# Eric-qi/NeuroQuant

Measured on AMD Instinct MI355X. Metric: calibration iters/sec (HNeRV Bunny 1280x640, 21k iters) + final PSNR vs ref, higher is better.
Workload: dtype f32 operands split into bf16 hi+lo, 3 BF16 MFMAs per product, fp32 accumulate (bf16x3); fp32 MFMA on small layers; 1 GPU; HNeRV Bunny_1280x640_3M, channel_wise, bits 6 5 4 5 5 6 6, phase-2 (AdaRound) iteration; per_gpu_batch=2, global_batch=2, frames=132, parallelism=dp1

## Files before the change

include/nq_hip.h:

```cpp
#ifndef NQ_HIP_H
#define NQ_HIP_H

#include <stdint.h>

#ifdef __cplusplus
extern "C" {
#endif

typedef void* nq_stream_t;

#define NQ_API __attribute__((visibility("default")))

#define NQ_OK 0
#define NQ_ERR_INVALID (-1)
#define NQ_ERR_UNSUPPORTED (-2)
#define NQ_ERR_LAUNCH (-3)

NQ_API int nq_abi_version(void);
NQ_API const char* nq_error_string(int code);


NQ_API int nq_scale_init_max(const float* x, int64_t rows, int64_t row_len, int n_levels, float* delta, float* zp,
                      nq_stream_t stream);

// ... 162 lines not shown
  float* db;
  int Cout, N, co_pad, n_pad, nsplit;
  int swap_kk;
  int sg;
} nq_wgr_seg;
NQ_API int nq_conv_wgrad3_slabs(const float* x, const float* dy, float* dw, float* db, float* ws, int B, int Cin, int H, int W, int Cout,
                         int k, nq_wgr_seg* seg, nq_stream_t stream);
NQ_API int nq_conv_wgrad3_slabs_fmt(const float* x, const float* dy, float* dw, float* db, float* ws, int B, int Cin, int H, int W,
                             int Cout, int k, nq_wgr_seg* seg, int fmt, nq_stream_t stream);
NQ_API int nq_conv_wgrad3_swapped_slabs(const float* x, const float* dy, float* dw, float* ws, int B, int Cin, int H, int W, int Cout,
                                 int k, nq_wgr_seg* seg, nq_stream_t stream);
NQ_API int nq_conv_wgrad_slabs(const float* x, const float* dy, float* dw, float* db, float* ws, int B, int Cin, int H, int W, int Cout,
                        int k, int x_gelu, nq_wgr_seg* seg, nq_stream_t stream);
NQ_API int nq_wgrad_reduce_multi(const nq_wgr_seg* segs, int nseg, nq_stream_t stream);

NQ_API int nq_ps_gelu_backward(const float* da, const float* z, float* dconv, int B, int C, int H, int W, int r,
                        nq_stream_t stream);

NQ_API int nq_tanh_out_backward(const float* dimg, const float* img, float* dconv, int64_t n, nq_stream_t stream);

NQ_API int nq_l2_loss(const float* pred, const float* tgt, float* loss, float* dpred, float* ws, int64_t n, int64_t mean_count,
               float gscale, nq_stream_t stream);

NQ_API int nq_channel_sum(const float* x, float* out, float* ws, int B, int C, int64_t HW, nq_stream_t stream);

NQ_API int nq_l2_loss_tanh_head(const float* pred, const float* tgt, const uint8_t* cache_u8, const int64_t* idx, float* loss,
                         float* dconv, float* db, float* ws, int B, int C, int64_t HW, int64_t mean_count, float gscale,
                         nq_stream_t stream);

NQ_API int64_t nq_head_forward_loss_ws_floats(int B, int H, int W);
// ... 22 lines not shown
```

neuroquant_amd/_lib.py:

```python
import ctypes
import os
from ctypes import c_char_p, c_float, c_int, c_int64, c_void_p, POINTER, Structure

_HERE = os.path.dirname(os.path.abspath(__file__))
LIB_PATH = os.environ.get("NQ_LIB") or os.path.join(_HERE, "libnqhip.so")

NQ_OK = 0
ABI_VERSION = 5
EPI_PLAIN, EPI_PS_GELU, EPI_TANH, EPI_PS, EPI_DGRAD_GELU = 0, 1, 2, 3, 4


class NQLibraryError(RuntimeError):
    pass


class AdaSeg(Structure):
    _fields_ = [("x", c_void_p), ("gy", c_void_p), ("alpha", c_void_p), ("delta", c_void_p), ("zp", c_void_p),
                ("out", c_void_p), ("rows", c_int64), ("row_len", c_int64), ("per_row", c_int), ("n_levels", c_int),
                ("soft", c_int), ("reg_weight", c_float)]


class WL3Seg(Structure):
    _fields_ = [("w", c_void_p), ("wt3", c_void_p), ("Cin", c_int), ("Cout", c_int), ("k", c_int), ("transposed", c_int)]

# ... 86 lines not shown
    sig("nq_weight_layout3", I, P, P, I, I, I, I, P)
    sig("nq_weight_layout3_multi", I, POINTER(WL3Seg), I, P)
    sig("nq_weight_layouts_multi", I, POINTER(WLSeg), I, P)
    sig("nq_weight_layouts_all", I, POINTER(WL3Seg), I, POINTER(WLSeg), I, P)
    sig("nq_conv_forward3_ws_floats", L, I, I, I, I, I, I)
    sig("nq_conv_forward3", I, P, P, P, P, P, P, P, I, I, I, I, I, I, I, I, P)
    sig("nq_conv_wgrad3_supported", I, I, I, I, I, I, I)
    sig("nq_conv_wgrad3_ws_floats", L, I, I, I, I, I, I)
    sig("nq_conv_wgrad3_plan", I, I, I, I, I, I, I, POINTER(c_int), POINTER(c_int), POINTER(c_int), POINTER(c_int))
    sig("nq_conv_wgrad3", I, P, P, P, P, P, I, I, I, I, I, I, P)
    sig("nq_conv_wgrad3_swapped", I, P, P, P, P, I, I, I, I, I, I, P)
    sig("nq_conv_wgrad3_slabs", I, P, P, P, P, P, I, I, I, I, I, I, POINTER(WgrSeg), P)
    sig("nq_conv_wgrad3_swapped_slabs", I, P, P, P, P, I, I, I, I, I, I, POINTER(WgrSeg), P)
    sig("nq_conv_wgrad_slabs", I, P, P, P, P, P, I, I, I, I, I, I, I, POINTER(WgrSeg), P)
    sig("nq_wgrad_reduce_multi", I, POINTER(WgrSeg), I, P)
    sig("nq_conv_wgrad_ws_floats", L, I, I, I, I, I, I)
    sig("nq_conv_wgrad", I, P, P, P, P, P, I, I, I, I, I, I, I, P)
    sig("nq_ps_gelu_backward", I, P, P, P, I, I, I, I, I, P)
    sig("nq_tanh_out_backward", I, P, P, P, L, P)
    sig("nq_l2_loss", I, P, P, P, P, P, L, L, F, P)
    sig("nq_channel_sum", I, P, P, P, I, I, L, P)
    sig("nq_l2_loss_tanh_head", I, P, P, P, P, P, P, P, P, I, I, L, L, F, P)
    sig("nq_frame_sse", I, P, P, P, L, L, P)
    sig("nq_ms_ssim_ws_floats", L, L, I, I, I)
    sig("nq_ms_ssim", I, P, P, P, P, L, I, I, I, P)
    sig("nq_gather_frames_u8", I, P, P, P, L, L, P)
    sig("nq_adaround_fwht_multi", I, POINTER(FqFwhtSeg), I, P)
    sig("nq_fwht_adaround_adam_multi", I, POINTER(FqFwhtSeg), I, F, F, F, F, F, F, P, P)
    sig("nq_head_forward_loss_ws_floats", L, I, I, I)
    sig("nq_head_forward_loss", I, P, P, I, P, P, P, P, P, P, P, P, P, I, I, I, I, L, F, P)
# ... 3 lines not shown
    return lib


EXPORTS = (
    "nq_abi_version", "nq_error_string", "nq_scale_init_max", "nq_uaq_forward", "nq_uaq_backward",
    "nq_adaround_init", "nq_adaround_forward", "nq_adaround_backward", "nq_reduce_ws_floats", "nq_round_loss", "nq_round_loss_backward",
    "nq_adam_step", "nq_adaround_adam_multi", "nq_adaround_forward_multi", "nq_uaq_forward_multi", "nq_uaq_backward_multi", "nq_adaround_backward_multi", "nq_adam_step_multi", "nq_step_prologue", "nq_step_prologue_gather", "nq_adaround_backward_multi_dyn", "nq_adam_step_multi_dyn", "nq_fwht", "nq_fwht_multi", "nq_weight_layouts", "nq_conv_operand_dims", "nq_conv_forward_ws_floats", "nq_conv_forward",
    "nq_conv3_supported", "nq_conv3_weight_bytes", "nq_weight_layout3", "nq_weight_layout3_multi", "nq_weight_layouts_multi", "nq_conv_forward3_ws_floats", "nq_conv_forward3",
    "nq_conv_wgrad3_supported", "nq_conv_wgrad3_ws_floats", "nq_conv_wgrad3_plan", "nq_conv_wgrad3", "nq_conv_wgrad3_swapped",
    "nq_conv_wgrad3_slabs", "nq_conv_wgrad3_swapped_slabs", "nq_conv_wgrad_slabs", "nq_wgrad_reduce_multi",
    "nq_conv_wgrad_ws_floats", "nq_conv_wgrad", "nq_ps_gelu_backward", "nq_tanh_out_backward", "nq_l2_loss",
    "nq_channel_sum", "nq_l2_loss_tanh_head", "nq_frame_sse", "nq_ms_ssim_ws_floats", "nq_ms_ssim", "nq_gather_frames_u8",
    "nq_act_dd", "nq_pixel_shuffle", "nq_bias_add", "nq_conv3_split_io", "nq_conv_split_out", "nq_split_words",
    "nq_conv_wgrad3_split_io", "nq_conv_wgrad3_fmt", "nq_conv_wgrad3_slabs_fmt", "nq_head_forward_loss_ws_floats", "nq_head_forward_loss",
    "nq_adaround_fwht_multi", "nq_fwht_adaround_adam_multi", "nq_weight_layouts_all",
)

_lib = None


def lib():
    global _lib
    if _lib is None:
        _lib = _load()
    return _lib


def check(rc, what=""):
    if rc != NQ_OK:
        msg = lib().nq_error_string(rc).decode()
# ... 2 lines not shown
```

neuroquant_amd/csrc/conv.hip:

```cpp
#include <algorithm>

#include "nq_common.h"

extern "C" {
int nq_tiny_pw_supported(int B, int Cin, int H, int W, int Cout, int k);
int nq_tiny_pw_forward(const float* x, const float* wt, const float* bias, float* y, float* z, const float* zprev, int B,
                       int Cin, int H, int W, int Cout, int ld, int r, int epi, hipStream_t st);
int nq_tiny_pw_wgrad(const float* x, const float* dy, float* dw, float* db, int B, int Cin, int H, int W, int Cout,
                     hipStream_t st);
}

extern "C" {
int nq_conv_igemm_k1(const float*, const float*, const float*, float*, float*, int, int, int, int, int, int, int, int, int,
                     int, float*, int, const float*, hipStream_t);
int nq_conv_igemm_k3(const float*, const float*, const float*, float*, float*, int, int, int, int, int, int, int, int, int,
                     int, float*, int, const float*, hipStream_t);
int nq_conv_igemm_k5(const float*, const float*, const float*, float*, float*, int, int, int, int, int, int, int, int, int,
                     int, float*, int, const float*, hipStream_t);
int nq_conv_splitk_finish(const float*, const float*, float*, float*, const float*, int, int, int, int, int, int, int,
                          hipStream_t);
int nq_head_supported(int, int);
int nq_head_forward(const float*, const float*, int, const float*, float*, int, int, int, int, int, int, int, hipStream_t);
int nq_head_dgrad(const float*, const float*, int, const float*, float*, int, int, int, int, int, int, int, int, hipStream_t);
int nq_head_dgrad_streams(int, int, int, int, int, int, int, int);
// ... 256 lines not shown
  const int mi = pick_mi_fwd(Cout);
  const int ns = pick_nsplit(B, Cin, H, W, Cout, k);
  if (ns > 1 && !ws) return NQ_ERR_INVALID;
  if ((int64_t)B * ns > 65535) return NQ_ERR_UNSUPPORTED;
  hipStream_t st = nq_s(stream);
  int rc;
  switch (k) {
    case 1: rc = nq_conv_igemm_k1(x, wt, bias, y, z, B, Cin, H, W, Cout, ld, r, epilogue, mi, ns, ws, in_gelu, zprev, st); break;
    case 3: rc = nq_conv_igemm_k3(x, wt, bias, y, z, B, Cin, H, W, Cout, ld, r, epilogue, mi, ns, ws, in_gelu, zprev, st); break;
    default: rc = nq_conv_igemm_k5(x, wt, bias, y, z, B, Cin, H, W, Cout, ld, r, epilogue, mi, ns, ws, in_gelu, zprev, st); break;
  }
  if (rc != NQ_OK || ns == 1) return rc;
  return nq_conv_splitk_finish(ws, bias, y, z, zprev, B, H, W, Cout, r, epilogue, ns, st);
}

int64_t nq_conv_wgrad_ws_floats(int B, int Cin, int H, int W, int Cout, int k) {
  if (!ks_ok(k) || B <= 0 || Cin <= 0 || H <= 0 || W <= 0 || Cout <= 0) return 0;
  WgradPlan p = plan_wgrad(B, Cin, H, W, Cout, k);
  return (int64_t)p.nsplit * p.co_pad * ((int64_t)p.n_pad + 1);
}

static int conv_wgrad_impl(const float* x, const float* dy, float* dw, float* db, float* ws, int B, int Cin, int H, int W,
                           int Cout, int k, int x_gelu, nq_wgr_seg* seg, nq_stream_t stream);

int nq_conv_wgrad(const float* x, const float* dy, float* dw, float* db, float* ws, int B, int Cin, int H, int W, int Cout,
                  int k, int x_gelu, nq_stream_t stream) {
  return conv_wgrad_impl(x, dy, dw, db, ws, B, Cin, H, W, Cout, k, x_gelu, nullptr, stream);
}

int nq_conv_wgrad_slabs(const float* x, const float* dy, float* dw, float* db, float* ws, int B, int Cin, int H, int W, int Cout,
// ... 36 lines not shown
```

neuroquant_amd/csrc/conv3.hip:

```cpp
#include <cstdlib>
#include "nq_common.h"
#include "conv3_layout.h"

extern "C" {
int nq_conv_igemm3_k3(const float*, const void*, const float*, float*, float*, const float*, int, int, int, int, int, int, int,
                      int, int, int, float*, hipStream_t);
int nq_conv_igemm3_k5(const float*, const void*, const float*, float*, float*, const float*, int, int, int, int, int, int, int,
                      int, int, int, float*, hipStream_t);
int nq_conv_splitk_finish(const float*, const float*, float*, float*, const float*, int, int, int, int, int, int, int, hipStream_t);
int nq_conv3_nst_k3();
int nq_conv3_nst_k5();
int nq_conv3_nst8_k3();
int nq_conv3_nst8_k5();
int nq_conv3_nstk_k3(int);
int nq_conv3_nstk_k5(int);
int nq_conv_flat3_plan(int, int, int, int, int, int, int*, int*, int*, int*);
int nq_conv_flat3(const float*, const void*, const float*, float*, float*, const float*, float*, int, int, int, int, int, int, int, int,
                  int, int, int, int, hipStream_t);
int nq_conv_wgrad_flat3_ok(int, int, int, int, int, int);
int nq_conv_wgrad_flat3(const float*, const float*, float*, float*, int, int, int, int, int, int, hipStream_t);
int nq_conv_wgrad3_k3(const float*, const float*, float*, float*, int, int, int, int, int, int, int, int, int, int, int, int, hipStream_t);
int nq_conv_wgrad3_k5(const float*, const float*, float*, float*, int, int, int, int, int, int, int, int, int, int, int, int, hipStream_t);
}

namespace {

constexpr int CC = 16;

inline int pick_mi3(int Cout) {
  if (Cout <= 16) return 1;
  if (Cout <= 32) return 2;
  int best = 3, best_pad = 1 << 30;
  for (int mi = 5; mi >= 3; --mi) {
    int mt = 16 * mi, pad = (Cout + mt - 1) / mt * mt;
    if (pad < best_pad) {
// ... 289 lines not shown
      } else {
        dw[i] = t;
      }
    } else if (db && i < total + Cout) {
      db[(int)(i - total)] = t;
    }
  }
}

constexpr int WGR_MAXSEG = 16;
struct WGRMulti {
  nq_wgr_seg s[WGR_MAXSEG];
  int blk0[WGR_MAXSEG + 1];
  int nseg;
};
__global__ __launch_bounds__(256) void wgrad_reduce_multi_kernel(WGRMulti t) {
  __shared__ float4 part[256];
  int k = 0;
  while (k + 1 < t.nseg && (int)blockIdx.x >= t.blk0[k + 1]) ++k;
  const nq_wgr_seg& q = t.s[k];
  const int SG = q.sg, OG = 256 / SG;
  const int o = threadIdx.x % OG, g = threadIdx.x / OG;
  const int N = q.N, Cout = q.Cout, nsplit = q.nsplit;
  const int NQ = (N + 3) >> 2;
  const int64_t i = (int64_t)((int)blockIdx.x - t.blk0[k]) * OG + o;
  const int64_t total = (int64_t)Cout * NQ;
  float4 s = make_float4(0.f, 0.f, 0.f, 0.f);
  int co = 0, n = 0;
  if (i < total) {
    co = (int)(i / NQ);
    n = 4 * (int)(i - (int64_t)co * NQ);
    const float* p = q.slab + (int64_t)co * q.n_pad + n;
    const int64_t stride = (int64_t)q.co_pad * q.n_pad;
#pragma unroll 8
    for (int j = g; j < nsplit; j += SG) {
      const float4 v = *reinterpret_cast<const float4*>(p + j * stride);
      s.x += v.x; s.y += v.y; s.z += v.z; s.w += v.w;
    }
  } else if (q.db && i < total + Cout) {
    const int cb = (int)(i - total);
// ... 17 lines not shown
      for (int e = 0; e < 4; ++e) {
        if (n + e >= N) break;
        const int ci = (n + e) / q.swap_kk, tap = (n + e) - ci * q.swap_kk;
        q.dw[((int64_t)ci * Cout + co) * q.swap_kk + (q.swap_kk - 1 - tap)] = sv[e];
      }
    } else if ((N & 3) == 0) {
      *reinterpret_cast<float4*>(q.dw + (int64_t)co * N + n) = s;
    } else {
#pragma unroll
      for (int e = 0; e < 4; ++e)
        if (n + e < N) q.dw[(int64_t)co * N + n + e] = sv[e];
    }
  } else if (q.db && i < total + Cout) {
    q.db[(int)(i - total)] = s.x;
  }
}

}

extern "C" {

int nq_conv3_supported(int B, int Cin, int H, int W, int Cout, int k) {
  if (!(k == 3 || k == 5) || B <= 0 || Cin <= 0 || Cout <= 4 || Cin <= 4) return 0;
  if ((int64_t)B * Cin * H * W * 4 >= 0xFFFFFF00ll) return 0;
  if (use_flat3(B, Cin, H, W, Cout, k, nullptr) && (int64_t)Cin * k * k * Cout >= 65536) return 1;
  const Fwd3Plan p = plan_fwd3(B, Cin, H, W, Cout);
  return p.wgs * p.nsplit >= 128;
}

int64_t nq_conv_forward3_ws_floats(int B, int Cin, int H, int W, int Cout, int k) {
// ... 181 lines not shown
  return conv_wgrad3_impl(dy, x, dw, nullptr, ws, B, Cout, H, W, Cin, k, k * k, nullptr, stream);
}

int nq_conv_wgrad3_slabs(const float* x, const float* dy, float* dw, float* db, float* ws, int B, int Cin, int H, int W, int Cout,
                         int k, nq_wgr_seg* seg, nq_stream_t stream) {
  if (!seg) return NQ_ERR_INVALID;
  return conv_wgrad3_impl(x, dy, dw, db, ws, B, Cin, H, W, Cout, k, 0, seg, stream);
}

int nq_conv_wgrad3_swapped_slabs(const float* x, const float* dy, float* dw, float* ws, int B, int Cin, int H, int W, int Cout,
                                 int k, nq_wgr_seg* seg, nq_stream_t stream) {
  if (!seg) return NQ_ERR_INVALID;
  return conv_wgrad3_impl(dy, x, dw, nullptr, ws, B, Cout, H, W, Cin, k, k * k, seg, stream);
}

int nq_wgrad_reduce_multi(const nq_wgr_seg* segs, int nseg, nq_stream_t stream) {
  if (!segs || nseg < 0) return NQ_ERR_INVALID;
  WGRMulti t;
  t.nseg = 0;
  int blocks = 0;
  auto flush = [&]() {
    if (t.nseg == 0) return;
    t.blk0[t.nseg] = blocks;
    hipLaunchKernelGGL(wgrad_reduce_multi_kernel, dim3((unsigned)blocks), dim3(256), 0, nq_s(stream), t);
    t.nseg = 0;
    blocks = 0;
  };
  for (int i = 0; i < nseg; ++i) {
    const nq_wgr_seg& h = segs[i];
    if (h.nsplit == 0) continue;
    if (!h.slab || !h.dw || h.Cout <= 0 || h.N <= 0 || h.nsplit < 0 || !(h.sg == 1 || h.sg == 4 || h.sg == 16) ||
        (h.db && !h.slab_db))
      return NQ_ERR_INVALID;
    if (t.nseg == WGR_MAXSEG) flush();
    t.s[t.nseg] = h;
    t.blk0[t.nseg] = blocks;
    const int og = 256 / h.sg;
    blocks += (int)(((int64_t)h.Cout * ((h.N + 3) / 4) + h.Cout + og - 1) / og);
    ++t.nseg;
  }
  flush();
  return nq_launch_status();
}

static int conv_wgrad3_impl(const float* x, const float* dy, float* dw, float* db, float* ws, int B, int Cin, int H, int W,
                            int Cout, int k, int swap_kk, nq_wgr_seg* seg, nq_stream_t stream, int fmt) {
  if (!x || !dy || !dw || !ws || B <= 0 || Cin <= 0 || H <= 0 || W <= 0 || Cout <= 0) return NQ_ERR_INVALID;
  if (!(k == 3 || k == 5)) return NQ_ERR_UNSUPPORTED;
  if ((int64_t)Cout * H * W >= (1ll << 31) || (int64_t)Cin * H * W >= (1ll << 31)) return NQ_ERR_UNSUPPORTED;
  if (swap_kk == 0 && nq_conv_wgrad_flat3_ok(B, Cin, H, W, Cout, k)) {
    if (fmt) return NQ_ERR_UNSUPPORTED;
    if (seg) *seg = nq_wgr_seg{nullptr, nullptr, dw, db, Cout, Cin * k * k, 0, 0, 0, 0, 1};
    return nq_conv_wgrad_flat3(x, dy, dw, db, B, Cin, H, W, Cout, k, nq_s(stream));
  }
  if (swap_kk != 0 && nq_conv_wgrad_flat3_ok(B, Cin, H, W, Cout, k)) return NQ_ERR_UNSUPPORTED;
// ... 26 lines not shown
```

neuroquant_amd/csrc/conv_tiny.hip:

```cpp
#include "nq_common.h"

namespace {

template <int KSL>
__global__ __launch_bounds__(256) void tiny_pw_fwd_kernel(const float* __restrict__ x, const float* __restrict__ wt,
                                                          const float* __restrict__ bias, float* __restrict__ y,
                                                          float* __restrict__ z, const float* __restrict__ zprev, int B,
                                                          int Cin, int H, int W, int Cout, int ld, int r, int epi) {
  constexpr int OPB = 256 / KSL;
  __shared__ float part[KSL][OPB];
  const int HW = H * W;
  const int o = threadIdx.x % OPB, ks = threadIdx.x / OPB;
  const int64_t t = (int64_t)blockIdx.x * OPB + o;
  const bool live = t < (int64_t)B * HW * Cout;
  const int co = live ? (int)(t % Cout) : 0, bp = live ? (int)(t / Cout) : 0;
  const int b = bp / HW, p = bp - b * HW;
  const float* __restrict__ xp = x + (int64_t)b * Cin * HW + p;
  float acc = 0.f;
#pragma unroll 8
  for (int ci = ks; ci < Cin; ci += KSL) acc = fmaf(wt[(int64_t)ci * ld + co], xp[(int64_t)ci * HW], acc);
  if (KSL > 1) {
    part[ks][o] = acc;
    __syncthreads();
    if (ks != 0) return;
    acc = part[0][o];
#pragma unroll
    for (int j = 1; j < KSL; ++j) acc += part[j][o];
  }
  if (!live) return;
  float v = acc + (bias ? bias[co] : 0.f);
  const int py = p / W, px = p - py * W;
  if (epi == NQ_EPI_PS_GELU || epi == NQ_EPI_PS) {
    const int rr = r * r, C = Cout / rr;
    const int c = co / rr, rem = co - c * rr, si = rem / r, sj = rem - si * r;
    const int64_t o = (((int64_t)b * C + c) * (H * r) + (int64_t)py * r + si) * ((int64_t)W * r) + (int64_t)px * r + sj;
    if (epi == NQ_EPI_PS_GELU) {
      float gv, dv;
      nq_gelu_pair(v, gv, dv);
      y[o] = gv;
      z[o] = dv;
    } else {
      z[o] = v;
    }
  } else if (epi == NQ_EPI_DGRAD_GELU) {
    const int64_t i = ((int64_t)b * Cout + co) * HW + p;
    v *= zprev[i];
    if (r == 1) {
      y[i] = v;
    } else {
      const int rr = r * r, yq = py / r, xq = px / r;
      const int ch = co * rr + (py - yq * r) * r + (px - xq * r);
      y[(((int64_t)b * Cout * rr + ch) * (H / r) + yq) * (int64_t)(W / r) + xq] = v;
    }
  } else {
    const int64_t i = ((int64_t)b * Cout + co) * HW + p;
    y[i] = (epi == NQ_EPI_TANH) ? tanhf(v) * 0.5f + 0.5f : v;
  }
}

__global__ __launch_bounds__(256) void tiny_pw_wgrad_kernel(const float* __restrict__ x, const float* __restrict__ dy,
                                                            float* __restrict__ dw, float* __restrict__ db, int B, int Cin,
                                                            int HW, int Cout) {
  const int64_t t = (int64_t)blockIdx.x * 256 + threadIdx.x;
  const int64_t nw = (int64_t)Cout * Cin;
  if (t < nw) {
    const int co = (int)(t / Cin), ci = (int)(t - (int64_t)co * Cin);
    float acc = 0.f;
    for (int b = 0; b < B; ++b) {
      const float* __restrict__ dp = dy + ((int64_t)b * Cout + co) * HW;
      const float* __restrict__ xp = x + ((int64_t)b * Cin + ci) * HW;
      if ((HW & 7) == 0) {
        for (int p = 0; p < HW; p += 8) {
          const float4 d0 = *reinterpret_cast<const float4*>(dp + p), d1 = *reinterpret_cast<const float4*>(dp + p + 4);
          const float4 x0 = *reinterpret_cast<const float4*>(xp + p), x1 = *reinterpret_cast<const float4*>(xp + p + 4);
          acc = fmaf(d0.x, x0.x, acc); acc = fmaf(d0.y, x0.y, acc); acc = fmaf(d0.z, x0.z, acc); acc = fmaf(d0.w, x0.w, acc);
          acc = fmaf(d1.x, x1.x, acc); acc = fmaf(d1.y, x1.y, acc); acc = fmaf(d1.z, x1.z, acc); acc = fmaf(d1.w, x1.w, acc);
        }
      } else {
        for (int p = 0; p < HW; ++p) acc = fmaf(dp[p], xp[p], acc);
      }
    }
    dw[t] = acc;
  } else if (db && t < nw + Cout) {
    const int co = (int)(t - nw);
    float acc = 0.f;
    for (int b = 0; b < B; ++b) {
      const float* __restrict__ dp = dy + ((int64_t)b * Cout + co) * HW;
      for (int p = 0; p < HW; ++p) acc += dp[p];
    }
    db[co] = acc;
  }
}

}

extern "C" {

int nq_tiny_pw_supported(int B, int Cin, int H, int W, int Cout, int k) {
  return k == 1 && (int64_t)B * H * W <= 256 && (int64_t)B * H * W * Cout < (1ll << 31);
}

int nq_tiny_pw_forward(const float* x, const float* wt, const float* bias, float* y, float* z, const float* zprev, int B,
                       int Cin, int H, int W, int Cout, int ld, int r, int epi, hipStream_t st) {
  const int64_t total = (int64_t)B * H * W * Cout;
  if (Cin > 1024)
    hipLaunchKernelGGL(tiny_pw_fwd_kernel<64>, dim3((unsigned)((total + 3) / 4)), dim3(256), 0, st, x, wt, bias, y, z, zprev,
                       B, Cin, H, W, Cout, ld, r, epi);
  else if (Cin > 256)
    hipLaunchKernelGGL(tiny_pw_fwd_kernel<16>, dim3((unsigned)((total + 15) / 16)), dim3(256), 0, st, x, wt, bias, y, z, zprev,
                       B, Cin, H, W, Cout, ld, r, epi);
  else if (Cin > 48)
    hipLaunchKernelGGL(tiny_pw_fwd_kernel<4>, dim3((unsigned)((total + 63) / 64)), dim3(256), 0, st, x, wt, bias, y, z, zprev,
                       B, Cin, H, W, Cout, ld, r, epi);
  else
    hipLaunchKernelGGL(tiny_pw_fwd_kernel<1>, dim3((unsigned)((total + 255) / 256)), dim3(256), 0, st, x, wt, bias, y, z, zprev,
                       B, Cin, H, W, Cout, ld, r, epi);
  return nq_launch_status();
}

int nq_tiny_pw_wgrad(const float* x, const float* dy, float* dw, float* db, int B, int Cin, int H, int W, int Cout,
                     hipStream_t st) {
  const int64_t total = (int64_t)Cout * Cin + (db ? Cout : 0);
  hipLaunchKernelGGL(tiny_pw_wgrad_kernel, dim3((unsigned)((total + 255) / 256)), dim3(256), 0, st, x, dy, dw, db, B, Cin,
                     H * W, Cout);
  return nq_launch_status();
}

}
```

neuroquant_amd/ops.py:

```python
import contextlib
import ctypes
import functools
import math
import os
import threading

import torch
from torch.autograd import Function

from . import _lib as L

_QCACHE = {}


def _q(name, *args):
    key = (name, args, os.environ.get("NQ_WGRAD3_PC"), os.environ.get("NQ_WGRAD3_SS"))
    v = _QCACHE.get(key)
    if v is None:
        v = _QCACHE[key] = getattr(L.lib(), name)(*args)
    return v

EPI_PLAIN, EPI_PS_GELU, EPI_TANH, EPI_PS, EPI_DGRAD_GELU = (L.EPI_PLAIN, L.EPI_PS_GELU, L.EPI_TANH, L.EPI_PS,
                                                                L.EPI_DGRAD_GELU)
EPI_X_SPLIT, EPI_Y_SPLIT = 0x100, 0x200


def _stream():
# ... 589 lines not shown
    ws = torch.empty(nws, device=x.device, dtype=torch.float32) if nws else None
    _timed(("conv_igemm3", k, cin, cout, H, W, B, epilogue),
           lambda: L.check(L.lib().nq_conv_forward3(_p(x), _p(wt3), _p(bias), _p(y), _p(z), _p(zprev), _p(ws), B, cin, H, W,
                                                    cout, k, r, epilogue | fmt, _stream()), "conv_forward3"))
    return y, z


def conv_wgrad3_supported(B, cin, H, W, cout, k):
    return bool(_q("nq_conv_wgrad3_supported", B, cin, H, W, cout, k))


class PendingReductions:

    def __init__(self):
        self.segs, self.keep = [], []

    def add(self, seg, *tensors):
        self.segs.append(seg)
        self.keep.append(tensors)

    def flush(self):
        if self.segs:
            arr = (L.WgrSeg * len(self.segs))(*self.segs)
            L.check(L.lib().nq_wgrad_reduce_multi(arr, len(self.segs), _stream()), "wgrad_reduce_multi")
        self.segs, self.keep = [], []


def conv_wgrad3_raw(x, dy, cout, k, want_db, out=None, defer=None, fmt=0):
    B, cin, H, W = x.shape
    ws = torch.empty(_q("nq_conv_wgrad3_ws_floats", B, cin, H, W, cout, k), device=x.device, dtype=torch.float32)
    dw = torch.empty((cout, cin, k, k), device=x.device, dtype=torch.float32) if out is None else out[0]
    db = (torch.empty(cout, device=x.device, dtype=torch.float32) if out is None else out[1]) if want_db else None
    if defer is not None:
        seg = L.WgrSeg()
        _timed(("conv_wgrad3", k, cin, cout, H, W, B, 0),
               lambda: L.check(L.lib().nq_conv_wgrad3_slabs_fmt(_p(x), _p(dy), _p(dw), _p(db), _p(ws), B, cin, H, W, cout, k,
                                                                ctypes.byref(seg), fmt, _stream()), "conv_wgrad3_slabs"))
# ... 28 lines not shown
        _timed(("conv_wgrad3", k, cout, cin, H, W, B, 0),
               lambda: L.check(L.lib().nq_conv_wgrad3_swapped_slabs(_p(x), _p(dy), _p(dw), _p(ws), B, cin, H, W, cout, k,
                                                                    ctypes.byref(seg), _stream()), "conv_wgrad3_swapped_slabs"))
        defer.add(seg, ws, dw)
    else:
        _timed(("conv_wgrad3", k, cout, cin, H, W, B, 0),
               lambda: L.check(L.lib().nq_conv_wgrad3_swapped(_p(x), _p(dy), _p(dw), _p(ws), B, cin, H, W, cout, k, _stream()),
                               "conv_wgrad3_swapped"))
    db = None
    if want_db:
        db = channel_sum(dy)
        if out is not None:
            out[1].copy_(db)
            db = out[1]
    return dw, db


def conv_wgrad_raw(x, dy, cout, k, want_db, x_gelu=False, out=None, defer=None):
    B, cin, H, W = x.shape
    ws = torch.empty(_q("nq_conv_wgrad_ws_floats", B, cin, H, W, cout, k), device=x.device, dtype=torch.float32)
    dw = torch.empty((cout, cin, k, k), device=x.device, dtype=torch.float32) if out is None else out[0]
    db = (torch.empty(cout, device=x.device, dtype=torch.float32) if out is None else out[1]) if want_db else None
    if defer is not None:
        seg = L.WgrSeg()
        _timed(("conv_wgrad", k, cin, cout, H, W, B, 0),
               lambda: L.check(L.lib().nq_conv_wgrad_slabs(_p(x), _p(dy), _p(dw), _p(db), _p(ws), B, cin, H, W, cout, k,
                                                           1 if x_gelu else 0, ctypes.byref(seg), _stream()), "conv_wgrad_slabs"))
        defer.add(seg, ws, dw, db)
        return dw, db
    _timed(("conv_wgrad", k, cin, cout, H, W, B, 0),
# ... 577 lines not shown
    def dgrad(l, dconv):
        k, r, act, cout, cin, in_gelu, wbk, dims_b, has_b, W3, x_split, g_split = metas[l]
        kp, rp, actp = spec.layers[l - 1]
        epi_b, r_b, zp = (EPI_DGRAD_GELU, rp, zs[l]) if actp else (EPI_PLAIN, 1, None)
        if not actp and rp != 1:
            raise NotImplementedError("PixelShuffle without activation between decoder layers")
        out_split = EPI_Y_SPLIT if metas[l - 1][11] else 0
        if W3 is not None:
            d, _ = conv3_forward_raw(dconv, W3, None, cin, k, epi_b, r_b, zprev=zp, fmt=(EPI_X_SPLIT if g_split else 0) | out_split)
        else:
            d, _ = conv_forward_raw(dconv, wbk, dims_b, None, cin, k, epi_b, r_b, zprev=zp, fmt=out_split)
        if not actp and l == 1 and spec.fc_hw != (1, 1):
            d = _channels_from_space(d, *spec.fc_hw).contiguous()
        return d

    def emb_grad(dconv):
        k, r, act, cout, cin, in_gelu, wbk, dims_b, has_b, W3 = metas[0][:10]
        return conv_forward_raw(dconv, wbk, dims_b, None, cin, k, EPI_PLAIN, 1)[0]

    if arena is not None and arena_two_phase and n > 1:
        dcs = [None] * n
        dcs[n - 1] = dconv
        for l in range(n - 1, 0, -1):
            dcs[l - 1] = dgrad(l, dcs[l])
        if ctx.needs_input_grad[0]:
            d_emb = emb_grad(dcs[0])
        flops = [metas[l][3] * metas[l][4] * metas[l][0] ** 2 * xs[l].shape[2] * xs[l].shape[3] for l in range(n)]
        split, late = n - 1, flops[n - 1]
        while split > 1 and late < 0.8 * sum(flops):
            split -= 1
# ... 2 lines not shown
            grads[2 * l], grads[2 * l + 1] = wgrad(l, dcs[l])
            dcs[l] = None
        off = sum(sizes[:2 * split])
        if pending is not None:
            pending.flush()
        yield arena[:off], False
        for l in range(split, n):
            grads[2 * l], grads[2 * l + 1] = wgrad(l, dcs[l])
            dcs[l] = None
        if pending is not None:
            pending.flush()
        yield arena[off:], True
        ctx.nq_arena_reduced = True
        return (d_emb, None) + tuple(grads)

    for l in range(n - 1, -1, -1):
        if side is not None:
            keep.append(dconv)
            side.wait_stream(main)
            with torch.cuda.stream(side):
                dw, db = wgrad(l, dconv)
            for t in (dw, db):
                if t is not None:
                    t.record_stream(main)
        else:
            dw, db = wgrad(l, dconv)
        grads[2 * l], grads[2 * l + 1] = dw, db
        if l == 0:
            if ctx.needs_input_grad[0]:
                d_emb = emb_grad(dconv)
            break
# ... 162 lines not shown
```

Baseline: 501.8 it/s (B=2 frames per iteration-equivalent, summed over GPUs).

## Fuse tiny pointwise dgrad with wgrad and fold first-layer wgrad into reduce

Adds a combined kernel that runs the tiny pointwise conv data-gradient and weight-gradient as separate block ranges of one launch. It also appends the first layer's tiny wgrad blocks onto the deferred slab-reduction kernel. Device bodies are moved into a shared header so several kernels can reuse them. The goal is fewer kernel launches and less serialization in the backward pass for small layers. The fused path is on by default behind an env flag and falls back when unsupported.

New measurement: 504.6 it/s (B=2 frames per iteration-equivalent, summed over GPUs), median of 3. About the same (+0.6%).

```diff
diff --git a/include/nq_hip.h b/include/nq_hip.h
--- a/include/nq_hip.h
+++ b/include/nq_hip.h
@@ -200,6 +200,13 @@
                         int k, int x_gelu, nq_wgr_seg* seg, nq_stream_t stream);
 NQ_API int nq_wgrad_reduce_multi(const nq_wgr_seg* segs, int nseg, nq_stream_t stream);
 
+NQ_API int nq_tiny_pw_supported(int B, int Cin, int H, int W, int Cout, int k);
+NQ_API int nq_conv_dgrad_wgrad_tiny(const float* x, const float* dy, float* dw, float* db, const float* wt_bwd, int krows, int ld,
+                             float* dx, const float* zprev, int B, int Cin, int H, int W, int Cout, int k, int r, int epilogue,
+                             nq_stream_t stream);
+NQ_API int nq_wgrad_reduce_multi_tiny(const nq_wgr_seg* segs, int nseg, const float* x, const float* dy, float* dw, float* db, int B,
+                               int Cin, int H, int W, int Cout, nq_stream_t stream);
+
 NQ_API int nq_ps_gelu_backward(const float* da, const float* z, float* dconv, int B, int C, int H, int W, int r,
                         nq_stream_t stream);
 
diff --git a/neuroquant_amd/_lib.py b/neuroquant_amd/_lib.py
--- a/neuroquant_amd/_lib.py
+++ b/neuroquant_amd/_lib.py
@@ -124,6 +124,9 @@
     sig("nq_conv_wgrad3_swapped_slabs", I, P, P, P, P, I, I, I, I, I, I, POINTER(WgrSeg), P)
     sig("nq_conv_wgrad_slabs", I, P, P, P, P, P, I, I, I, I, I, I, I, POINTER(WgrSeg), P)
     sig("nq_wgrad_reduce_multi", I, POINTER(WgrSeg), I, P)
+    sig("nq_tiny_pw_supported", I, I, I, I, I, I, I)
+    sig("nq_conv_dgrad_wgrad_tiny", I, P, P, P, P, P, I, I, P, P, I, I, I, I, I, I, I, I, P)
+    sig("nq_wgrad_reduce_multi_tiny", I, POINTER(WgrSeg), I, P, P, P, P, I, I, I, I, I, P)
     sig("nq_conv_wgrad_ws_floats", L, I, I, I, I, I, I)
     sig("nq_conv_wgrad", I, P, P, P, P, P, I, I, I, I, I, I, I, P)
     sig("nq_ps_gelu_backward", I, P, P, P, I, I, I, I, I, P)
@@ -157,6 +160,7 @@
     "nq_act_dd", "nq_pixel_shuffle", "nq_bias_add", "nq_conv3_split_io", "nq_conv_split_out", "nq_split_words",
     "nq_conv_wgrad3_split_io", "nq_conv_wgrad3_fmt", "nq_conv_wgrad3_slabs_fmt", "nq_head_forward_loss_ws_floats", "nq_head_forward_loss",
     "nq_adaround_fwht_multi", "nq_fwht_adaround_adam_multi", "nq_weight_layouts_all",
+    "nq_tiny_pw_supported", "nq_conv_dgrad_wgrad_tiny", "nq_wgrad_reduce_multi_tiny",
 )
 
 _lib = None
diff --git a/neuroquant_amd/csrc/conv.hip b/neuroquant_amd/csrc/conv.hip
--- a/neuroquant_amd/csrc/conv.hip
+++ b/neuroquant_amd/csrc/conv.hip
@@ -8,6 +8,8 @@
                        int Cin, int H, int W, int Cout, int ld, int r, int epi, hipStream_t st);
 int nq_tiny_pw_wgrad(const float* x, const float* dy, float* dw, float* db, int B, int Cin, int H, int W, int Cout,
                      hipStream_t st);
+int nq_tiny_pw_dgrad_wgrad(const float* x, const float* dy, float* dw, float* db, const float* wt_bwd, float* dx,
+                           const float* zprev, int B, int Cin, int H, int W, int Cout, int ld, int r, int epi, hipStream_t st);
 }
 
 extern "C" {
@@ -294,6 +296,22 @@
   return nq_conv_splitk_finish(ws, bias, y, z, zprev, B, H, W, Cout, r, epilogue, ns, st);
 }
 
+int nq_conv_dgrad_wgrad_tiny(const float* x, const float* dy, float* dw, float* db, const float* wt_bwd, int krows, int ld, float* dx,
+                             const float* zprev, int B, int Cin, int H, int W, int Cout, int k, int r, int epilogue,
+                             nq_stream_t stream) {
+  if (!x || !dy || !dw || !wt_bwd || !dx || B <= 0 || Cin <= 0 || H <= 0 || W <= 0 || Cout <= 0) return NQ_ERR_INVALID;
+  if (!ks_ok(k)) return NQ_ERR_UNSUPPORTED;
+  if (epilogue != NQ_EPI_PLAIN && epilogue != NQ_EPI_DGRAD_GELU) return NQ_ERR_INVALID;
+  if (epilogue == NQ_EPI_DGRAD_GELU && (!zprev || r <= 0 || H % r != 0 || W % r != 0)) return NQ_ERR_INVALID;
+  int need_rows, need_ld;
+  nq_conv_operand_dims(Cout, Cin, k, &need_rows, &need_ld);
+  if (krows < need_rows || ld < need_ld || (ld & 3)) return NQ_ERR_INVALID;
+  if (!nq_tiny_pw_supported(B, Cin, H, W, Cout, k) || !nq_tiny_pw_supported(B, Cout, H, W, Cin, k) ||
+      use_head_fwd(Cin, k, epilogue, 0) || use_head_dgrad(Cout, k, epilogue, 0, nullptr))
+    return NQ_ERR_UNSUPPORTED;
+  return nq_tiny_pw_dgrad_wgrad(x, dy, dw, db, wt_bwd, dx, zprev, B, Cin, H, W, Cout, ld, r, epilogue, nq_s(stream));
+}
+
 int64_t nq_conv_wgrad_ws_floats(int B, int Cin, int H, int W, int Cout, int k) {
   if (!ks_ok(k) || B <= 0 || Cin <= 0 || H <= 0 || W <= 0 || Cout <= 0) return 0;
   WgradPlan p = plan_wgrad(B, Cin, H, W, Cout, k);
diff --git a/neuroquant_amd/csrc/conv3.hip b/neuroquant_amd/csrc/conv3.hip
--- a/neuroquant_amd/csrc/conv3.hip
+++ b/neuroquant_amd/csrc/conv3.hip
@@ -1,6 +1,7 @@
 #include <cstdlib>
 #include "nq_common.h"
 #include "conv3_layout.h"
+#include "conv_tiny_impl.h"
 
 extern "C" {
 int nq_conv_igemm3_k3(const float*, const void*, const float*, float*, float*, const float*, int, int, int, int, int, int, int,
@@ -19,6 +20,7 @@
                   int, int, int, int, hipStream_t);
 int nq_conv_wgrad_flat3_ok(int, int, int, int, int, int);
 int nq_conv_wgrad_flat3(const float*, const float*, float*, float*, int, int, int, int, int, int, hipStream_t);
+int nq_tiny_pw_supported(int, int, int, int, int, int);
 int nq_conv_wgrad3_k3(const float*, const float*, float*, float*, int, int, int, int, int, int, int, int, int, int, int, int, hipStream_t);
 int nq_conv_wgrad3_k5(const float*, const float*, float*, float*, int, int, int, int, int, int, int, int, int, int, int, int, hipStream_t);
 }
@@ -338,16 +340,16 @@
   int blk0[WGR_MAXSEG + 1];
   int nseg;
 };
-__global__ __launch_bounds__(256) void wgrad_reduce_multi_kernel(WGRMulti t) {
+__device__ __forceinline__ void wgrad_reduce_multi_body(const WGRMulti& t, const int bx) {
   __shared__ float4 part[256];
   int k = 0;
-  while (k + 1 < t.nseg && (int)blockIdx.x >= t.blk0[k + 1]) ++k;
+  while (k + 1 < t.nseg && bx >= t.blk0[k + 1]) ++k;
   const nq_wgr_seg& q = t.s[k];
   const int SG = q.sg, OG = 256 / SG;
   const int o = threadIdx.x % OG, g = threadIdx.x / OG;
   const int N = q.N, Cout = q.Cout, nsplit = q.nsplit;
   const int NQ = (N + 3) >> 2;
-  const int64_t i = (int64_t)((int)blockIdx.x - t.blk0[k]) * OG + o;
+  const int64_t i = (int64_t)(bx - t.blk0[k]) * OG + o;
   const int64_t total = (int64_t)Cout * NQ;
   float4 s = make_float4(0.f, 0.f, 0.f, 0.f);
   int co = 0, n = 0;
@@ -395,6 +397,16 @@
   } else if (q.db && i < total + Cout) {
     q.db[(int)(i - total)] = s.x;
   }
+}
+
+__global__ __launch_bounds__(256) void wgrad_reduce_multi_kernel(WGRMulti t) { wgrad_reduce_multi_body(t, (int)blockIdx.x); }
+
+__global__ __launch_bounds__(256) void wgrad_reduce_multi_tiny_kernel(WGRMulti t, TinyWgArgs g) {
+  const int red_blocks = t.blk0[t.nseg];
+  if ((int)blockIdx.x < red_blocks)
+    wgrad_reduce_multi_body(t, (int)blockIdx.x);
+  else
+    tiny_pw_wgrad_body((int)blockIdx.x - red_blocks, g.x, g.dy, g.dw, g.db, g.B, g.Cin, g.HW, g.Cout);
 }
 
 }
@@ -606,8 +618,22 @@
   return conv_wgrad3_impl(dy, x, dw, nullptr, ws, B, Cout, H, W, Cin, k, k * k, seg, stream);
 }
 
+static int wgrad_reduce_multi_impl(const nq_wgr_seg* segs, int nseg, const TinyWgArgs* tiny, nq_stream_t stream);
+
 int nq_wgrad_reduce_multi(const nq_wgr_seg* segs, int nseg, nq_stream_t stream) {
   if (!segs || nseg < 0) return NQ_ERR_INVALID;
+  return wgrad_reduce_multi_impl(segs, nseg, nullptr, stream);
+}
+
+int nq_wgrad_reduce_multi_tiny(const nq_wgr_seg* segs, int nseg, const float* x, const float* dy, float* dw, float* db, int B,
+                               int Cin, int H, int W, int Cout, nq_stream_t stream) {
+  if ((nseg > 0 && !segs) || nseg < 0 || !x || !dy || !dw || B <= 0 || Cin <= 0 || H <= 0 || W <= 0 || Cout <= 0) return NQ_ERR_INVALID;
+  if (!nq_tiny_pw_supported(B, Cin, H, W, Cout, 1)) return NQ_ERR_UNSUPPORTED;
+  const TinyWgArgs g{x, dy, dw, db, B, Cin, H * W, Cout};
+  return wgrad_reduce_multi_impl(segs, nseg, &g, stream);
+}
+
+static int wgrad_reduce_multi_impl(const nq_wgr_seg* segs, int nseg, const TinyWgArgs* tiny, nq_stream_t stream) {
   WGRMulti t;
   t.nseg = 0;
   int blocks = 0;
@@ -631,6 +657,13 @@
     blocks += (int)(((int64_t)h.Cout * ((h.N + 3) / 4) + h.Cout + og - 1) / og);
     ++t.nseg;
   }
+  if (tiny) {
+    t.blk0[t.nseg] = blocks;
+    const int64_t tb = ((int64_t)tiny->Cout * tiny->Cin + (tiny->db ? tiny->Cout : 0) + 255) / 256;
+    if (blocks + tb >= (1ll << 31)) return NQ_ERR_UNSUPPORTED;
+    hipLaunchKernelGGL(wgrad_reduce_multi_tiny_kernel, dim3((unsigned)(blocks + tb)), dim3(256), 0, nq_s(stream), t, *tiny);
+    return nq_launch_status();
+  }
   flush();
   return nq_launch_status();
 }
diff --git a/neuroquant_amd/csrc/conv_tiny.hip b/neuroquant_amd/csrc/conv_tiny.hip
--- a/neuroquant_amd/csrc/conv_tiny.hip
+++ b/neuroquant_amd/csrc/conv_tiny.hip
@@ -1,4 +1,5 @@
 #include "nq_common.h"
+#include "conv_tiny_impl.h"
 
 namespace {
 
@@ -7,89 +8,30 @@
                                                           const float* __restrict__ bias, float* __restrict__ y,
                                                           float* __restrict__ z, const float* __restrict__ zprev, int B,
                                                           int Cin, int H, int W, int Cout, int ld, int r, int epi) {
-  constexpr int OPB = 256 / KSL;
-  __shared__ float part[KSL][OPB];
-  const int HW = H * W;
-  const int o = threadIdx.x % OPB, ks = threadIdx.x / OPB;
-  const int64_t t = (int64_t)blockIdx.x * OPB + o;
-  const bool live = t < (int64_t)B * HW * Cout;
-  const int co = live ? (int)(t % Cout) : 0, bp = live ? (int)(t / Cout) : 0;
-  const int b = bp / HW, p = bp - b * HW;
-  const float* __restrict__ xp = x + (int64_t)b * Cin * HW + p;
-  float acc = 0.f;
-#pragma unroll 8
-  for (int ci = ks; ci < Cin; ci += KSL) acc = fmaf(wt[(int64_t)ci * ld + co], xp[(int64_t)ci * HW], acc);
-  if (KSL > 1) {
-    part[ks][o] = acc;
-    __syncthreads();
-    if (ks != 0) return;
-    acc = part[0][o];
-#pragma unroll
-    for (int j = 1; j < KSL; ++j) acc += part[j][o];
-  }
-  if (!live) return;
-  float v = acc + (bias ? bias[co] : 0.f);
-  const int py = p / W, px = p - py * W;
-  if (epi == NQ_EPI_PS_GELU || epi == NQ_EPI_PS) {
-    const int rr = r * r, C = Cout / rr;
-    const int c = co / rr, rem = co - c * rr, si = rem / r, sj = rem - si * r;
-    const int64_t o = (((int64_t)b * C + c) * (H * r) + (int64_t)py * r + si) * ((int64_t)W * r) + (int64_t)px * r + sj;
-    if (epi == NQ_EPI_PS_GELU) {
-      float gv, dv;
-      nq_gelu_pair(v, gv, dv);
-      y[o] = gv;
-      z[o] = dv;
-    } else {
-      z[o] = v;
-    }
-  } else if (epi == NQ_EPI_DGRAD_GELU) {
-    const int64_t i = ((int64_t)b * Cout + co) * HW + p;
-    v *= zprev[i];
-    if (r == 1) {
-      y[i] = v;
-    } else {
-      const int rr = r * r, yq = py / r, xq = px / r;
-      const int ch = co * rr + (py - yq * r) * r + (px - xq * r);
-      y[(((int64_t)b * Cout * rr + ch) * (H / r) + yq) * (int64_t)(W / r) + xq] = v;
-    }
-  } else {
-    const int64_t i = ((int64_t)b * Cout + co) * HW + p;
-    y[i] = (epi == NQ_EPI_TANH) ? tanhf(v) * 0.5f + 0.5f : v;
-  }
+  tiny_pw_fwd_body<KSL>((int)blockIdx.x, x, wt, bias, y, z, zprev, B, Cin, H, W, Cout, ld, r, epi);
 }
 
 __global__ __launch_bounds__(256) void tiny_pw_wgrad_kernel(const float* __restrict__ x, const float* __restrict__ dy,
                                                             float* __restrict__ dw, float* __restrict__ db, int B, int Cin,
                                                             int HW, int Cout) {
-  const int64_t t = (int64_t)blockIdx.x * 256 + threadIdx.x;
-  const int64_t nw = (int64_t)Cout * Cin;
-  if (t < nw) {
-    const int co = (int)(t / Cin), ci = (int)(t - (int64_t)co * Cin);
-    float acc = 0.f;
-    for (int b = 0; b < B; ++b) {
-      const float* __restrict__ dp = dy + ((int64_t)b * Cout + co) * HW;
-      const float* __restrict__ xp = x + ((int64_t)b * Cin + ci) * HW;
-      if ((HW & 7) == 0) {
-        for (int p = 0; p < HW; p += 8) {
-          const float4 d0 = *reinterpret_cast<const float4*>(dp + p), d1 = *reinterpret_cast<const float4*>(dp + p + 4);
-          const float4 x0 = *reinterpret_cast<const float4*>(xp + p), x1 = *reinterpret_cast<const float4*>(xp + p + 4);
-          acc = fmaf(d0.x, x0.x, acc); acc = fmaf(d0.y, x0.y, acc); acc = fmaf(d0.z, x0.z, acc); acc = fmaf(d0.w, x0.w, acc);
-          acc = fmaf(d1.x, x1.x, acc); acc = fmaf(d1.y, x1.y, acc); acc = fmaf(d1.z, x1.z, acc); acc = fmaf(d1.w, x1.w, acc);
-        }
-      } else {
-        for (int p = 0; p < HW; ++p) acc = fmaf(dp[p], xp[p], acc);
-      }
-    }
-    dw[t] = acc;
-  } else if (db && t < nw + Cout) {
-    const int co = (int)(t - nw);
-    float acc = 0.f;
-    for (int b = 0; b < B; ++b) {
-      const float* __restrict__ dp = dy + ((int64_t)b * Cout + co) * HW;
-      for (int p = 0; p < HW; ++p) acc += dp[p];
-    }
-    db[co] = acc;
-  }
+  tiny_pw_wgrad_body((int)blockIdx.x, x, dy, dw, db, B, Cin, HW, Cout);
+}
+
+struct TinyFwdArgs {
+  const float* x;
+  const float* wt;
+  const float* bias;
+  float* y;
+  float* z;
+  const float* zprev;
+  int B, Cin, H, W, Cout, ld, r, epi;
+};
+template <int KSL>
+__global__ __launch_bounds__(256) void tiny_pw_dgrad_wgrad_kernel(TinyFwdArgs f, TinyWgArgs g, int fwd_blocks) {
+  if ((int)blockIdx.x < fwd_blocks)
+    tiny_pw_fwd_body<KSL>((int)blockIdx.x, f.x, f.wt, f.bias, f.y, f.z, f.zprev, f.B, f.Cin, f.H, f.W, f.Cout, f.ld, f.r, f.epi);
+  else
+    tiny_pw_wgrad_body((int)blockIdx.x - fwd_blocks, g.x, g.dy, g.dw, g.db, g.B, g.Cin, g.HW, g.Cout);
 }
 
 }
@@ -118,6 +60,24 @@
   return nq_launch_status();
 }
 
+int nq_tiny_pw_dgrad_wgrad(const float* x, const float* dy, float* dw, float* db, const float* wt_bwd, float* dx,
+                           const float* zprev, int B, int Cin, int H, int W, int Cout, int ld, int r, int epi, hipStream_t st) {
+  const int64_t total = (int64_t)B * H * W * Cin;
+  const int ksl = Cout > 1024 ? 64 : (Cout > 256 ? 16 : (Cout > 48 ? 4 : 1)), opb = 256 / ksl;
+  const int64_t fb = (total + opb - 1) / opb, wb = ((int64_t)Cout * Cin + (db ? Cout : 0) + 255) / 256;
+  if (fb + wb >= (1ll << 31)) return NQ_ERR_UNSUPPORTED;
+  const TinyFwdArgs f{dy, wt_bwd, nullptr, dx, nullptr, zprev, B, Cout, H, W, Cin, ld, r, epi};
+  const TinyWgArgs g{x, dy, dw, db, B, Cin, H * W, Cout};
+  const dim3 grid((unsigned)(fb + wb));
+  switch (ksl) {
+    case 64: hipLaunchKernelGGL(tiny_pw_dgrad_wgrad_kernel<64>, grid, dim3(256), 0, st, f, g, (int)fb); break;
+    case 16: hipLaunchKernelGGL(tiny_pw_dgrad_wgrad_kernel<16>, grid, dim3(256), 0, st, f, g, (int)fb); break;
+    case 4: hipLaunchKernelGGL(tiny_pw_dgrad_wgrad_kernel<4>, grid, dim3(256), 0, st, f, g, (int)fb); break;
+    default: hipLaunchKernelGGL(tiny_pw_dgrad_wgrad_kernel<1>, grid, dim3(256), 0, st, f, g, (int)fb); break;
+  }
+  return nq_launch_status();
+}
+
 int nq_tiny_pw_wgrad(const float* x, const float* dy, float* dw, float* db, int B, int Cin, int H, int W, int Cout,
                      hipStream_t st) {
   const int64_t total = (int64_t)Cout * Cin + (db ? Cout : 0);
diff --git a/neuroquant_amd/csrc/conv_tiny_impl.h b/neuroquant_amd/csrc/conv_tiny_impl.h
--- /dev/null
+++ b/neuroquant_amd/csrc/conv_tiny_impl.h
@@ -0,0 +1,104 @@
+#pragma once
+#include "nq_common.h"
+
+namespace {
+
+template <int KSL>
+__device__ __forceinline__ void tiny_pw_fwd_body(int bx, const float* __restrict__ x, const float* __restrict__ wt,
+                                                 const float* __restrict__ bias, float* __restrict__ y, float* __restrict__ z,
+                                                 const float* __restrict__ zprev, int B, int Cin, int H, int W, int Cout,
+                                                 int ld, int r, int epi) {
+  constexpr int OPB = 256 / KSL;
+  __shared__ float part[KSL][OPB];
+  const int HW = H * W;
+  const int o = threadIdx.x % OPB, ks = threadIdx.x / OPB;
+  const int64_t t = (int64_t)bx * OPB + o;
+  const bool live = t < (int64_t)B * HW * Cout;
+  const int co = live ? (int)(t % Cout) : 0, bp = live ? (int)(t / Cout) : 0;
+  const int b = bp / HW, p = bp - b * HW;
+  const float* __restrict__ xp = x + (int64_t)b * Cin * HW + p;
+  float acc = 0.f;
+#pragma unroll 8
+  for (int ci = ks; ci < Cin; ci += KSL) acc = fmaf(wt[(int64_t)ci * ld + co], xp[(int64_t)ci * HW], acc);
+  if (KSL > 1) {
+    part[ks][o] = acc;
+    __syncthreads();
+    if (ks != 0) return;
+    acc = part[0][o];
+#pragma unroll
+    for (int j = 1; j < KSL; ++j) acc += part[j][o];
+  }
+  if (!live) return;
+  float v = acc + (bias ? bias[co] : 0.f);
+  const int py = p / W, px = p - py * W;
+  if (epi == NQ_EPI_PS_GELU || epi == NQ_EPI_PS) {
+    const int rr = r * r, C = Cout / rr;
+    const int c = co / rr, rem = co - c * rr, si = rem / r, sj = rem - si * r;
+    const int64_t o = (((int64_t)b * C + c) * (H * r) + (int64_t)py * r + si) * ((int64_t)W * r) + (int64_t)px * r + sj;
+    if (epi == NQ_EPI_PS_GELU) {
+      float gv, dv;
+      nq_gelu_pair(v, gv, dv);
+      y[o] = gv;
+      z[o] = dv;
+    } else {
+      z[o] = v;
+    }
+  } else if (epi == NQ_EPI_DGRAD_GELU) {
+    const int64_t i = ((int64_t)b * Cout + co) * HW + p;
+    v *= zprev[i];
+    if (r == 1) {
+      y[i] = v;
+    } else {
+      const int rr = r * r, yq = py / r, xq = px / r;
+      const int ch = co * rr + (py - yq * r) * r + (px - xq * r);
+      y[(((int64_t)b * Cout * rr + ch) * (H / r) + yq) * (int64_t)(W / r) + xq] = v;
+    }
+  } else {
+    const int64_t i = ((int64_t)b * Cout + co) * HW + p;
+    y[i] = (epi == NQ_EPI_TANH) ? tanhf(v) * 0.5f + 0.5f : v;
+  }
+}
+
+__device__ __forceinline__ void tiny_pw_wgrad_body(int bx, const float* __restrict__ x, const float* __restrict__ dy,
+                                                   float* __restrict__ dw, float* __restrict__ db, int B, int Cin, int HW,
+                                                   int Cout) {
+  const int64_t t = (int64_t)bx * 256 + threadIdx.x;
+  const int64_t nw = (int64_t)Cout * Cin;
+  if (t < nw) {
+    const int co = (int)(t / Cin), ci = (int)(t - (int64_t)co * Cin);
+    float acc = 0.f;
+    for (int b = 0; b < B; ++b) {
+      const float* __restrict__ dp = dy + ((int64_t)b * Cout + co) * HW;
+      const float* __restrict__ xp = x + ((int64_t)b * Cin + ci) * HW;
+      if ((HW & 7) == 0) {
+        for (int p = 0; p < HW; p += 8) {
+          const float4 d0 = *reinterpret_cast<const float4*>(dp + p), d1 = *reinterpret_cast<const float4*>(dp + p + 4);
+          const float4 x0 = *reinterpret_cast<const float4*>(xp + p), x1 = *reinterpret_cast<const float4*>(xp + p + 4);
+          acc = fmaf(d0.x, x0.x, acc); acc = fmaf(d0.y, x0.y, acc); acc = fmaf(d0.z, x0.z, acc); acc = fmaf(d0.w, x0.w, acc);
+          acc = fmaf(d1.x, x1.x, acc); acc = fmaf(d1.y, x1.y, acc); acc = fmaf(d1.z, x1.z, acc); acc = fmaf(d1.w, x1.w, acc);
+        }
+      } else {
+        for (int p = 0; p < HW; ++p) acc = fmaf(dp[p], xp[p], acc);
+      }
+    }
+    dw[t] = acc;
+  } else if (db && t < nw + Cout) {
+    const int co = (int)(t - nw);
+    float acc = 0.f;
+    for (int b = 0; b < B; ++b) {
+      const float* __restrict__ dp = dy + ((int64_t)b * Cout + co) * HW;
+      for (int p = 0; p < HW; ++p) acc += dp[p];
+    }
+    db[co] = acc;
+  }
+}
+
+struct TinyWgArgs {
+  const float* x;
+  const float* dy;
+  float* dw;
+  float* db;
+  int B, Cin, HW, Cout;
+};
+
+}
diff --git a/neuroquant_amd/ops.py b/neuroquant_amd/ops.py
--- a/neuroquant_amd/ops.py
+++ b/neuroquant_amd/ops.py
@@ -11,6 +11,7 @@
 from . import _lib as L
 
 _QCACHE = {}
+_FOLD = os.environ.get("NQ_FOLD", "1") != "0"
 
 
 def _q(name, *args):
@@ -630,13 +631,25 @@
 
     def __init__(self):
         self.segs, self.keep = [], []
+        self.tiny = None
 
     def add(self, seg, *tensors):
         self.segs.append(seg)
         self.keep.append(tensors)
 
+    def add_tiny(self, x, dy, dw, db, cout):
+        assert self.tiny is None
+        self.tiny = (x, dy, dw, db, cout)
+
     def flush(self):
-        if self.segs:
+        if self.tiny is not None:
+            x, dy, dw, db, cout = self.tiny
+            B, cin, H, W = x.shape
+            arr = (L.WgrSeg * max(1, len(self.segs)))(*self.segs)
+            L.check(L.lib().nq_wgrad_reduce_multi_tiny(arr, len(self.segs), _p(x), _p(dy), _p(dw), _p(db), B, cin, H, W, cout,
+                                                       _stream()), "wgrad_reduce_multi_tiny")
+            self.tiny = None
+        elif self.segs:
             arr = (L.WgrSeg * len(self.segs))(*self.segs)
             L.check(L.lib().nq_wgrad_reduce_multi(arr, len(self.segs), _stream()), "wgrad_reduce_multi")
         self.segs, self.keep = [], []
@@ -695,6 +708,27 @@
             out[1].copy_(db)
             db = out[1]
     return dw, db
+
+
+def tiny_pw_supported(B, cin, H, W, cout, k):
+    return bool(_q("nq_tiny_pw_supported", B, cin, H, W, cout, k))
+
+
+def conv_dgrad_wgrad_tiny(x, dy, wbk, dims_b, cout, k, want_db, epilogue, r, zprev=None, out=None):
+    B, cin, H, W = x.shape
+    dw = torch.empty((cout, cin, k, k), device=x.device, dtype=torch.float32) if out is None else out[0]
+    db = (torch.empty(cout, device=x.device, dtype=torch.float32) if out is None else out[1]) if want_db else None
+    if epilogue == EPI_DGRAD_GELU:
+        dx = torch.empty((B, cin * r * r, H // r, W // r), device=x.device, dtype=torch.float32)
+    else:
+        dx = torch.empty((B, cin, H, W), device=x.device, dtype=torch.float32)
+    rc = _timed(("conv_wgrad_dgrad", k, cin, cout, H, W, B, epilogue),
+                lambda: L.lib().nq_conv_dgrad_wgrad_tiny(_p(x), _p(dy), _p(dw), _p(db), _p(wbk), dims_b[0], dims_b[1], _p(dx),
+                                                         _p(zprev), B, cin, H, W, cout, k, r, epilogue, _stream()))
+    if rc == -2:
+        return None
+    L.check(rc, "conv_dgrad_wgrad_tiny")
+    return dw, db, dx
 
 
 def conv_wgrad_raw(x, dy, cout, k, want_db, x_gelu=False, out=None, defer=None):
@@ -1302,6 +1336,25 @@
             d = _channels_from_space(d, *spec.fc_hw).contiguous()
         return d
 
+    def wgrad_dgrad(l, dconv):
+        k, r, act, cout, cin, in_gelu, wbk, dims_b, has_b, W3, x_split, g_split = metas[l]
+        kp, rp, actp = spec.layers[l - 1]
+        if in_gelu or x_split or g_split or metas[l - 1][11] or (not actp and rp != 1) or (l == n - 1 and head_db is not None):
+            return None
+        epi_b, r_b, zp = (EPI_DGRAD_GELU, rp, zs[l]) if actp else (EPI_PLAIN, 1, None)
+        x_in = xs[l]
+        Bx, _, Hx, Wx = x_in.shape
+        out = views[l] if views is not None else None
+        res = None
+        if W3 is None and wbk is not None and tiny_pw_supported(Bx, cin, Hx, Wx, cout, k) and tiny_pw_supported(Bx, cout, Hx, Wx, cin, k):
+            res = conv_dgrad_wgrad_tiny(x_in, dconv, wbk, dims_b, cout, k, has_b, epi_b, r_b, zprev=zp, out=out)
+        if res is None:
+            return None
+        dw, db, d = res
+        if not actp and l == 1 and spec.fc_hw != (1, 1):
+            d = _channels_from_space(d, *spec.fc_hw).contiguous()
+        return dw, db, d
+
     def emb_grad(dconv):
         k, r, act, cout, cin, in_gelu, wbk, dims_b, has_b, W3 = metas[0][:10]
         return conv_forward_raw(dconv, wbk, dims_b, None, cin, k, EPI_PLAIN, 1)[0]
@@ -1334,7 +1387,24 @@
         ctx.nq_arena_reduced = True
         return (d_emb, None) + tuple(grads)
 
+    fold = _FOLD and side is None
     for l in range(n - 1, -1, -1):
+        both = wgrad_dgrad(l, dconv) if fold and l > 0 else None
+        if both is not None:
+            grads[2 * l], grads[2 * l + 1], dconv = both
+            continue
+        if fold and l == 0 and pending is not None:
+            k, r, act, cout, cin, in_gelu = metas[0][:6]
+            x_in = xs[0]
+            if not in_gelu and tiny_pw_supported(x_in.shape[0], cin, x_in.shape[2], x_in.shape[3], cout, k):
+                out = views[0] if views is not None else None
+                dw = torch.empty((cout, cin, k, k), device=g.device, dtype=torch.float32) if out is None else out[0]
+                db = (torch.empty(cout, device=g.device, dtype=torch.float32) if out is None else out[1]) if metas[0][8] else None
+                pending.add_tiny(x_in, dconv, dw, db, cout)
+                grads[0], grads[1] = dw, db
+                if ctx.needs_input_grad[0]:
+                    d_emb = emb_grad(dconv)
+                break
         if side is not None:
             keep.append(dconv)
             side.wait_stream(main)
```
